# Moon0shang/HandPoseEstimation-with-3D-CNNs

Measured on AMD Instinct MI355X. Metric: depth frames/sec to 32^3 TSDF, higher is better.
Workload: dtype f64

## Files before the change

### handposeestimation-with-3d-cnns_amd/csrc/abi.inc

```


extern "C" {

void tsdf_default_cam(tsdf_cam *cam) {
  if (cam) *cam = kDefaultCam;
}

int tsdf_version(void) { return TSDF_ABI_VERSION; }

const char *tsdf_strerror(int status) {
  switch (status) {
    case TSDF_OK: return "ok";
    case TSDF_ERR_INVALID_ARG: return "invalid argument";
    case TSDF_ERR_NO_DEVICE: return "no usable HIP device (this library is gfx950-only and has no CPU fallback)";
    case TSDF_ERR_LAUNCH: return "HIP kernel launch failed";
    default: return "unknown tsdf status";
  }
}

int tsdf_resolution_supported(int R) { return R >= 4 && R <= kMaxR && (R % 4) == 0; }

int tsdf_voxelize_hip(const float *d_depth, int64_t depth_len, const int64_t *d_offsets, const int32_t *d_headers, int n,
                      int R, const tsdf_cam *cam, int layout, void *hip_stream, float *d_out_tsdf,
                      float *d_out_max_l, float *d_out_mid_p, int32_t *d_out_status) {
// ... 123 lines not shown
}

int tsdf_voxelize_indexed_pca_hip(const float *d_depth, int64_t depth_len, const int64_t *d_offsets,
                                  const int32_t *d_headers, int64_t n_pack, const int64_t *d_index, int n, int R,
                                  const tsdf_cam *cam, int layout, void *hip_stream, const double *d_xforms,
                                  float *d_out_tsdf, float *d_out_max_l, float *d_out_mid_p, int32_t *d_out_status,
                                  const tsdf_labels *labels, const tsdf_pca *pca) {
  RunOpts o;
  o.needs = kNeedPlacement | kNeedIndex | kNeedLabels | kNeedPca;
  o.labels = labels;
  o.index = d_index;
  o.n_src = n_pack;
  o.xforms = d_xforms;
  o.pca = pca;
  return run(Frames{d_depth, depth_len, d_offsets, d_headers, n, R, cam, layout, hip_stream},
             Outs{d_out_tsdf, d_out_max_l, d_out_mid_p, d_out_status}, o);
}

int tsdf_voxelize_indexed_host_pca_hip(const float *d_depth, int64_t depth_len, const int64_t *d_offsets,
                                       const int32_t *d_headers, int64_t n_pack, const int64_t *h_index, int n, int R,
                                       const tsdf_cam *cam, int layout, void *hip_stream, float *d_out_tsdf,
                                       float *d_out_max_l, float *d_out_mid_p, int32_t *d_out_status,
                                       const tsdf_labels *labels, const tsdf_pca *pca) {
  RunOpts o;
  o.needs = kNeedPlacement | kNeedHostIndex | kNeedLabels | kNeedPca;
  o.labels = labels;
  o.h_index = h_index;
  o.n_src = n_pack;
  o.pca = pca;
  return run(Frames{d_depth, depth_len, d_offsets, d_headers, n, R, cam, layout, hip_stream},
             Outs{d_out_tsdf, d_out_max_l, d_out_mid_p, d_out_status}, o);
}

int tsdf_project_joints_hip(const float *d_gt, const float *d_max_l, const float *d_mid_p, int n, int n_joints,
                            const tsdf_pca *pca, void *hip_stream) {
  return run_project(d_gt, d_max_l, d_mid_p, n, n_joints, pca, hip_stream);
}

int tsdf_pose_error_hip(const float *d_pred, const tsdf_pca *pca, const float *d_max_l, const float *d_mid_p,
                        const float *d_gt, int n, int n_joints, void *hip_stream, float *d_out_err,
                        float *d_out_frame_mean, float *d_out_frame_max, float *d_out_joints) {
  return run_pose_error(d_pred, pca, d_max_l, d_mid_p, d_gt, n, n_joints, hip_stream, d_out_err, d_out_frame_mean,
                        d_out_frame_max, d_out_joints);
}

int tsdf_point_clouds_hip(const float *d_depth, int64_t depth_len, const int64_t *d_offsets, const int32_t *d_headers,
                          int n, int points, const tsdf_cam *cam, uint64_t seed, int64_t frame_base,
                          const double *d_xforms, void *hip_stream, double *d_out_points, int32_t *d_out_count,
                          int32_t *d_out_status) {
  return run_point_clouds(d_depth, depth_len, d_offsets, d_headers, n, points, cam, seed, frame_base, d_xforms,
                          hip_stream, d_out_points, d_out_count, d_out_status);
}

int tsdf_cloud_grid_hip(const double *d_points, int n, int points, int R, const tsdf_cam *cam, void *hip_stream,
                        float *d_out_grid, float *d_out_max_l, float *d_out_mid_p, float *d_out_aabb,
                        int32_t *d_out_status) {
  return run_cloud_grid(d_points, n, points, R, cam, hip_stream, d_out_grid, d_out_max_l, d_out_mid_p, d_out_aabb,
                        d_out_status);
}

#ifdef TSDF_DEBUG_HOOKS
int tsdf_debug_pixmap_hip(const float *d_depth, int64_t depth_len, const int64_t *d_offsets, const int32_t *d_headers,
                          int n, int R, const tsdf_cam *cam, int layout, void *hip_stream, const float *d_grid,
                          float *d_out_tsdf, int32_t *d_out_pixmap, int32_t *d_out_status) {
  RunOpts o;
  o.needs = kNeedPixmap;
  o.grid_in = d_grid;
  o.pixmap = d_out_pixmap;
  return run(Frames{d_depth, depth_len, d_offsets, d_headers, n, R, cam, layout, hip_stream},
             Outs{d_out_tsdf, nullptr, nullptr, d_out_status}, o);
}
#endif

int tsdf_stream_release(void *hip_stream) {
  int dev = 0;
  if (hipGetDevice(&dev) != hipSuccess) {
    (void)hipGetLastError();
    return TSDF_OK;
  }
  (void)stream_slot(dev, static_cast<hipStream_t>(hip_stream), true);
  return TSDF_OK;
}

#ifdef TSDF_DEBUG_HOOKS
int tsdf_debug_set_queue_word(void *hip_stream, uint64_t value) {
  int dev = 0;
  const int rc = check_device(&dev);
  if (rc != TSDF_OK) return rc;
  hipStream_t s = static_cast<hipStream_t>(hip_stream);
  const int i = stream_slot(dev, s, false);
  if (i < 0) return TSDF_ERR_INVALID_ARG;
  if (hipStreamSynchronize(s) != hipSuccess) return TSDF_ERR_LAUNCH;
  const unsigned long long v = value;
  if (hipMemcpy(g_slots[dev].base + i, &v, sizeof v, hipMemcpyHostToDevice) != hipSuccess) return TSDF_ERR_LAUNCH;
  return TSDF_OK;
}
#endif

int tsdf_describe_launch(int n, int R, int layout, int aug, char *buf, int buflen) {
  if (!buf || buflen < 1 || n < 1 || !tsdf_resolution_supported(R)) return TSDF_ERR_INVALID_ARG;
  if (layout != TSDF_LAYOUT_CZYX && layout != TSDF_LAYOUT_CXYZ) return TSDF_ERR_INVALID_ARG;
  int dev = 0;
  const int rc = check_device(&dev);
  if (rc != TSDF_OK) return rc;
  const int rt = (R == 32 || R == 64) ? R : 0;
  int S = 0, per = R;
  split_plan(n, R, num_cus(), &S, &per);
  if (S >= 2) {
    snprintf(buf, (size_t)buflen, "tsdf_split_kernel<%d, %d, %s, x%d", rt, layout, aug ? "true" : "false", S);
  } else {
    snprintf(buf, (size_t)buflen, "tsdf_fused_kernel<%d, %d, %s, false, %d>", rt, layout, aug ? "true" : "false",
             groups_for(R));
  }
  return TSDF_OK;
}

#ifdef TSDF_STAMPS
int tsdf_debug_read_stamps(unsigned long long *host_out, int count) {
  const int total = kStampBlocks * kStampFrames * kStampSlots;
  if (count > total) count = total;
  if (hipDeviceSynchronize() != hipSuccess) return -1;
  if (hipMemcpyFromSymbol(host_out, HIP_SYMBOL(g_stamps), sizeof(unsigned long long) * count) != hipSuccess)
    return -1;
  return count;
}
int tsdf_debug_read_wstamps(unsigned long long *host_out, int count) {
  const int total = kStampBlocks * kStampFrames * 16 * 2;
  if (count > total) count = total;
  if (hipDeviceSynchronize() != hipSuccess) return -1;
  if (hipMemcpyFromSymbol(host_out, HIP_SYMBOL(g_wstamps), sizeof(unsigned long long) * count) != hipSuccess)
    return -1;
  return count;
}
#endif

}
```

### handposeestimation-with-3d-cnns_amd/csrc/frame.inc

```

struct KArgs {
  const float *depth;
  const int64_t *offsets;
  const int32_t *headers;
  int n, R;
  CamK cam;
  float *tsdf, *max_l, *mid_p;
  int32_t *status;
  float *aabb, *grid, *ori;
  int aabb_only;
  const float *grid_in;
  unsigned long long *queue;
  unsigned int qepoch;
  const double *xforms;
  int64_t depth_len;
  const int64_t *index;
  int64_t n_src;
  int n_inline;
  int64_t inline_index[TSDF_INLINE_INDEX_MAX];
  const float *gt;
  float *gt_nor, *gt_aug;
  int n_joints, clamp;
  int32_t *pixmap;
  int split, per;
  float *xchg;
  unsigned int seq;
  int polls;
  const float *pca_mean, *pca_coeff;
  float *gt_pca;
  int pca_k;
};

struct FrameHdr {
  int frame;
  int l, t, r, b;
  int pad;
  int64_t off0, off1;
  int64_t src;
};

__device__ __forceinline__ void fetch_header(const KArgs &a, const int64_t *__restrict__ in_offsets,
                                             const int32_t *__restrict__ in_headers, int fr, FrameHdr &m) {
  int64_t src = fr;
  bool ok = true;
  if (a.n_inline) {
    src = a.inline_index[fr];
    ok = src >= 0 && src < a.n_src;
    if (!ok) src = 0;
  } else if (a.index) {
    src = a.index[fr];
    ok = src >= 0 && src < a.n_src;
    if (!ok) src = 0;
  }
  const int32_t *h = in_headers + 6 * src;
  m.l = h[2];
  m.t = h[3];
  m.r = h[4];
  m.b = h[5];
  m.off0 = in_offsets[src];
  m.off1 = ok ? in_offsets[src + 1] : m.off0 - 1;
  m.src = src;
}

struct HelpReq {
  Grid g;
  VoxK vk;
  const float *src;
  float *out;
  int frame, use_tab, mode, owner;
  int pm_bw, pm_dc, pm_dr, pad;
};

struct GroupCtl {
  int bar[kMaxGroups];
  int local_next;
  int tile_next;
  int lock;
  int help_for;
  int idle[kMaxGroups];
  int cap_fail[kMaxGroups];
  FrameHdr hdr[kMaxGroups];
  HelpReq help;
};


__device__ __forceinline__ int lds_load(const int *p) {
  return __hip_atomic_load(p, __ATOMIC_RELAXED, __HIP_MEMORY_SCOPE_WORKGROUP);
}
__device__ __forceinline__ void lds_store(int *p, int v) {
  __hip_atomic_store(p, v, __ATOMIC_RELAXED, __HIP_MEMORY_SCOPE_WORKGROUP);
}

template <int GWAVES>
__device__ __forceinline__ void group_barrier(int *cnt, int &target) {
  target += GWAVES;
  asm volatile("s_waitcnt lgkmcnt(0)" ::: "memory");
  if ((threadIdx.x & 63) == 0) {
    __hip_atomic_fetch_add(cnt, 1, __ATOMIC_RELAXED, __HIP_MEMORY_SCOPE_WORKGROUP);
    while (__hip_atomic_load(cnt, __ATOMIC_RELAXED, __HIP_MEMORY_SCOPE_WORKGROUP) < target)
      __builtin_amdgcn_s_sleep(1);
  }
  asm volatile("" ::: "memory");
}

template <int RT, bool AUG, int GROUPS = 2>
struct Lds {
  static constexpr int kZ = RT ? RT : kMaxR;
  static constexpr bool kHasTab = !AUG && (RT == 0 || RT <= kTabR);
  static constexpr int kTabN = kHasTab ? kTabR * kTabR : 16;
  struct PerGroup {
    alignas(16) unsigned pytab[kTabN];
    alignas(16) int pxtab[kTabN];
    alignas(16) unsigned char pyrow[kTabN];
    alignas(16) ZEntry ztab[kZ];
    alignas(16) double atab[AUG ? 12 * kZ : 2];
    alignas(16) unsigned rowtab[kMaxRows];
    alignas(16) float red[16 * kRedStride];
  };
  static constexpr int kFixed = GROUPS * (int)sizeof(PerGroup) + (int)sizeof(GroupCtl) + 64;
  static constexpr int kPoolFloats = ((kLdsBytes - kFixed) / 16) * 4;
  static constexpr int kPoolUnits = kPoolFloats / 4;
  static_assert(kPoolUnits < 16384, "pool offsets are 14 bits of 4-float units");
  struct Block {
    alignas(16) float pool[kPoolFloats];
    PerGroup pg[GROUPS];
    alignas(16) GroupCtl ctl;
  };
  static_assert(sizeof(Block) <= kLdsBytes, "LDS layout exceeds the CU");
};

template <class PG>
__device__ __forceinline__ Tabs make_tabs(PG &pg) {
  Tabs t;
  t.ztab = (LdsZ)pg.ztab;
  t.pxtab = (LdsCI)pg.pxtab;
  t.pytab = (LdsCU)pg.pytab;
  t.pyrow = (LdsCU8)pg.pyrow;
  t.rowtab = (LdsCU)pg.rowtab;
  t.atab = (LdsCD)pg.atab;
  return t;
}

__device__ __forceinline__ bool frame_from_header(const FrameHdr &fh, const float *depth, int64_t depth_len, Frame &f) {
  f.l = __builtin_amdgcn_readfirstlane(fh.l);
  f.t = __builtin_amdgcn_readfirstlane(fh.t);
  f.r = __builtin_amdgcn_readfirstlane(fh.r);
  f.b = __builtin_amdgcn_readfirstlane(fh.b);
  const int64_t bw = (int64_t)f.r - f.l, bh = (int64_t)f.b - f.t;
  f.bw = (int)bw;
  f.bh = (int)bh;
  f.depth = depth + fh.off0;
  return bw > 0 && bh > 0 && bw <= 0x7fffffff && bh <= 0x7fffffff && bw * bh == fh.off1 - fh.off0 && fh.off0 >= 0 &&
         fh.off1 <= depth_len;
}

__device__ __forceinline__ bool finite32(float v) { return __builtin_fabsf(v) < TSDF_INF; }

__device__ __forceinline__ void place_grid(Aabb &ab, int R, const CamK &cam, const float *grid_in, int frame,
                                           Grid &g, int &status) {
  if (!ab.any) {
    status = TSDF_FRAME_DEGENERATE;
    ab.mn[0] = ab.mn[1] = ab.mn[2] = ab.mx[0] = ab.mx[1] = ab.mx[2] = 0.f;
    return;
  }
  g = glue(ab.mn, ab.mx, R, cam);
// ... 236 lines not shown
```

### handposeestimation-with-3d-cnns_amd/csrc/kernels.inc

```

template <int RT, int LAYOUT, bool AUG, bool DBG, int GROUPS, bool PCA>
__global__ __launch_bounds__(kWG) void tsdf_fused_kernel(const KArgs a, const float *__restrict__ in_depth,
                                                         const int64_t *__restrict__ in_offsets,
                                                         const int32_t *__restrict__ in_headers,
                                                         const double *__restrict__ in_xforms) {
  constexpr int kGroups = GROUPS, kGW = kWG / GROUPS, kGWaves = kGW / 64;
  using L = Lds<RT, AUG, GROUPS>;
  __shared__ typename L::Block lds;

  const int R = RT ? RT : a.R;
  const CamK &cam = a.cam;
  const int n = a.n;
  const int tid = threadIdx.x, lane = tid & 63, gtid = tid & (kGW - 1);
  const int group = __builtin_amdgcn_readfirstlane(tid / kGW);
  const int gwave = __builtin_amdgcn_readfirstlane((tid >> 6) & (kGWaves - 1));
  auto &pg = lds.pg[group];
  GroupCtl &ctl = lds.ctl;

  if (tid == 0) {
    for (int i = 0; i < kGroups; ++i) ctl.bar[i] = ctl.idle[i] = ctl.cap_fail[i] = 0;
    ctl.lock = 0;
    ctl.help_for = 0;
    ctl.local_next = kGroups;
  }
  __syncthreads();
  int bar_target = 0;
  auto gsync = [&]() { group_barrier<kGWaves>(&ctl.bar[group], bar_target); };

  Capture cap;
  cap.pool = (LdsF)lds.pool;
  cap.rowtab = (LdsU)pg.rowtab;
  cap.fail = (LdsI)&ctl.cap_fail[group];
  cap.cap4 = 0;
  cap.base4 = 0;
  cap.on = false;

  const int n_static = gridDim.x * kGroups;

  int iter = 0;
  (void)iter;
  for (;; ++iter) {
    if (gwave == 0) {
      int fr;
      if (iter == 0) {
        fr = blockIdx.x + gridDim.x * group;
      } else if (a.queue) {
        unsigned int t = 0;
        if (lane == 0) {
          t = queue_ticket(a.queue, a.qepoch, n);
        }
        fr = n_static + (int)__builtin_amdgcn_readfirstlane(t);
      } else {
        int t = 0;
        if (lane == 0) t = __hip_atomic_fetch_add(&ctl.local_next, 1, __ATOMIC_RELAXED, __HIP_MEMORY_SCOPE_WORKGROUP);
        const int64_t f64i = (int64_t)blockIdx.x + (int64_t)gridDim.x * __builtin_amdgcn_readfirstlane(t);
        fr = f64i < n ? (int)f64i : n;
      }
      FrameHdr m;
      m.frame = fr < n ? fr : -1;
      m.l = m.t = m.r = m.b = m.pad = 0;
      m.off0 = m.off1 = m.src = 0;
      if (fr < n) fetch_header(a, in_offsets, in_headers, fr, m);
      if (lane == 0) {
        ctl.hdr[group] = m;
        ctl.cap_fail[group] = 0;
      }
    }
    gsync();
    const FrameHdr fh = ctl.hdr[group];
    const int frame = __builtin_amdgcn_readfirstlane(fh.frame);
    if (frame < 0) break;
    TSDF_STAMP(kGroups * iter + group, 0);

    Frame f;
    const bool hdr_ok = frame_from_header(fh, in_depth, a.depth_len, f);
    float *out = a.tsdf ? a.tsdf + (int64_t)frame * 3 * R * R * R : nullptr;
    const bool want_vol = !a.aabb_only && out;

    int status = TSDF_FRAME_OK;
    Aabb ab;
    ab.any = false;
    ab.mn[0] = ab.mn[1] = ab.mn[2] = ab.mx[0] = ab.mx[1] = ab.mx[2] = 0.f;
    ab.c0 = ab.r0 = 0;
    ab.c1 = ab.r1 = -1;
    Grid g;
    g.mid[0] = g.mid[1] = g.mid[2] = 0.f;
    g.max_l = g.voxel_len = g.trunc = 0.f;
    g.ori[0] = g.ori[1] = g.ori[2] = 0.f;
    const double *xf = AUG ? in_xforms + 24 * (int64_t)frame : nullptr;

    bool holds_lock = false;
    if (!hdr_ok) {
      status = TSDF_FRAME_BAD_HEADER;
    } else {
      float fin[kExt];
      auto sync_ext = [&]() {
        if (want_vol && gwave == 0 && lane == 0) {
          while (atomicCAS(&ctl.lock, 0, 1) != 0) __builtin_amdgcn_s_sleep(2);
        }
        gsync();
      };
      phase1_extents<kGWaves, AUG, false>(f, cam, 0, f.bh, pg.red, fin, gwave, sync_ext, cap, kGroups * iter + group, xf);
      holds_lock = want_vol;
      ab = aabb_from_extents(fin);
      TSDF_STAMP(kGroups * iter + group, 4);
      place_grid(ab, R, cam, a.grid_in, frame, g, status);
    }

    if (gtid == 0) write_frame_outputs(a, frame, g, ab, status);
    write_labels<PCA>(a, frame, fh.src, g, status, xf, gtid, kGW);

    if (want_vol) {
      if (status != TSDF_FRAME_OK) {
        zero_volume(out, R, gtid, kGW, 0, 1);
        if constexpr (DBG) {
          if (a.pixmap)
            for (int i = gtid; i < R * R * R; i += kGW) a.pixmap[(int64_t)frame * R * R * R + i] = -1;
        }
      } else {
        int vt = gtid;
        asm volatile("" : "+v"(vt));
        int mode = kFillGlobal;
        const int sc0 = DBG ? 0 : ab.c0, sr0 = DBG ? 0 : ab.r0;
        const int sw = DBG ? f.bw : ab.c1 - ab.c0 + 1, sh = DBG ? f.bh : ab.r1 - ab.r0 + 1;
        const int sw4 = (sw + 3) & ~3;
        const bool staged = (int64_t)sw4 * sh <= L::kPoolFloats;
        if (staged) {
          mode = kFillRect;
          stage_rect_dma<kGWaves>(lds.pool, f, fh.off1 - fh.off0, sc0, sr0, sh, sw4, gwave, lane);
        }
        const VoxK vk = make_voxk(cam, g, f, ab, mode, DBG, sw4);
        const bool use_tab = !AUG && R <= kTabR;
        TSDF_STAMP(kGroups * iter + group, 5);
        fill_tables<LAYOUT, AUG>(pg, g, cam, vk, R, use_tab, false, xf, vt, kGW);
        TSDF_STAMP(kGroups * iter + group, 6);
        if (staged) asm volatile("s_waitcnt vmcnt(0)" ::: "memory");
        TSDF_STAMP(kGroups * iter + group, 7);
        if constexpr (kGroups == 2) {
          if (gwave == 0 && lane == 0) ctl.hdr[group].pad = lds_load(&ctl.idle[group ^ 1]);
        }
        if constexpr (kGroups == 1) {
          if (gwave == 0 && lane == 0) lds_store(&ctl.tile_next, 0);
        }
        gsync();
        TSDF_STAMP(kGroups * iter + group, 8);
        bool helped = false;
        if constexpr (kGroups == 2) {
          if (__builtin_amdgcn_readfirstlane(ctl.hdr[group].pad)) {
            helped = true;
            if (gwave == 0 && lane == 0) {
              HelpReq hq;
              hq.g = g;
              hq.vk = vk;
              hq.src = f.depth + vk.base;
              hq.mode = mode;
              hq.owner = group;
              hq.out = out;
              hq.frame = frame;
              hq.use_tab = use_tab;
              hq.pm_bw = f.bw;
              hq.pm_dc = vk.px0 - f.l;
              hq.pm_dr = vk.py0 - f.t;
              hq.pad = 0;
              ctl.help = hq;
              lds_store(&ctl.help_for, (group ^ 1) + 1);
            }
          }
        }
        TSDF_STAMP_VAL(kGroups * iter + group, 10, helped ? 2 : 1);
        const Tabs tb = make_tabs(pg);
        PixMapK pm;
        pm.out = DBG && a.pixmap ? (GlobalPix)(a.pixmap + (int64_t)frame * R * R * R) : (GlobalPix) nullptr;
        pm.bw = f.bw;
        pm.dc = vk.px0 - f.l;
        pm.dr = vk.py0 - f.t;
        auto run2 = [&](auto src) {
          if constexpr (kGroups == 2) {
            if (__builtin_expect(helped, 0)) {
              if constexpr (AUG) {
                phase2_aug<LAYOUT, 2 * kGW>(g, cam, vk, R, xf, tb, src, (GlobalOut)out, vt, 0, R);
              } else {
                phase2<LAYOUT, 2 * kGW, DBG>(g, cam, vk, R, tb, use_tab, src, (GlobalOut)out, vt, 0, R, pm);
              }
              return;
            }
          }
          if constexpr (AUG) {
            phase2_aug<LAYOUT, kGW>(g, cam, vk, R, xf, tb, src, (GlobalOut)out, vt, 0, R,
                                    kGroups == 1 ? &ctl.tile_next : nullptr, kGroups * iter + group);
          } else {
            phase2<LAYOUT, kGW, DBG>(g, cam, vk, R, tb, use_tab, src, (GlobalOut)out, vt, 0, R, pm,
                                     kGroups == 1 ? &ctl.tile_next : nullptr);
          }
        };
        if (mode == kFillRect) {
          run2(LdsRect{(LdsSrc)lds.pool});
        } else {
          run2((GlobalSrc)(f.depth + vk.base));
        }
      }
    }
    TSDF_STAMP(kGroups * iter + group, 9);
    gsync();
    if (holds_lock && gwave == 0 && lane == 0)
      __hip_atomic_store(&ctl.lock, 0, __ATOMIC_RELAXED, __HIP_MEMORY_SCOPE_WORKGROUP);
  }
  if constexpr (kGroups == 2) {
    if (gwave == 0 && lane == 0) {
      lds_store(&ctl.idle[group], 1);
      int dec;
      for (;;) {
        if (lds_load(&ctl.help_for) == group + 1) { dec = 1; break; }
        if (lds_load(&ctl.idle[group ^ 1])) { dec = lds_load(&ctl.help_for) == group + 1; break; }
        __builtin_amdgcn_s_sleep(8);
      }
      ctl.hdr[group].pad = dec;
    }
    gsync();
    if (__builtin_amdgcn_readfirstlane(ctl.hdr[group].pad)) {
      const HelpReq hq = ctl.help;
      const GlobalOut hout = (GlobalOut)hq.out;
      const GlobalSrc hsrc = (GlobalSrc)hq.src;
      const Tabs tb = make_tabs(lds.pg[group ^ 1]);
      PixMapK pm;
      pm.out = DBG && a.pixmap ? (GlobalPix)(a.pixmap + (int64_t)hq.frame * R * R * R) : (GlobalPix) nullptr;
      pm.bw = hq.pm_bw;
      pm.dc = hq.pm_dc;
      pm.dr = hq.pm_dr;
      auto run2 = [&](auto src) {
        if constexpr (AUG) {
          phase2_aug<LAYOUT, 2 * kGW>(hq.g, cam, hq.vk, R, in_xforms + 24 * (int64_t)hq.frame, tb, src, hout,
                                      kGW + gtid, 0, R);
        } else {
          phase2<LAYOUT, 2 * kGW, DBG>(hq.g, cam, hq.vk, R, tb, hq.use_tab != 0, src, hout, kGW + gtid, 0, R, pm);
        }
      };
      if (hq.mode == kFillRect) {
        run2(LdsRect{(LdsSrc)lds.pool});
      } else {
        run2(hsrc);
      }
    }
  }
}


template <int RT, int LAYOUT, bool AUG, bool XCHG, bool PCA>
__global__ __launch_bounds__(kWG) void tsdf_split_kernel(const KArgs a, const float *__restrict__ in_depth,
                                                         const int64_t *__restrict__ in_offsets,
                                                         const int32_t *__restrict__ in_headers,
                                                         const double *__restrict__ in_xforms) {
  using L = Lds<RT, AUG>;
  __shared__ typename L::Block lds;

  const int R = RT ? RT : a.R;
  const CamK &cam = a.cam;
  const int tid = threadIdx.x;
  const int wave = __builtin_amdgcn_readfirstlane(tid >> 6);
  const int frame = blockIdx.x / a.split, part = blockIdx.x - frame * a.split;
  auto &pg = lds.pg[0];
  GroupCtl &ctl = lds.ctl;
  if (tid == 0) ctl.cap_fail[0] = 0;
  FrameHdr fh;
  {
    fh.frame = frame;
    fh.pad = 0;
    fetch_header(a, in_offsets, in_headers, frame, fh);
  }
  __syncthreads();
  TSDF_STAMP(0, 0);
  Frame f;
  const bool hdr_ok = frame_from_header(fh, in_depth, a.depth_len, f);
  float *out = a.tsdf ? a.tsdf + (int64_t)frame * 3 * R * R * R : nullptr;
  const bool want_vol = !a.aabb_only && out;

  int status = TSDF_FRAME_OK;
  Aabb ab;
  ab.any = false;
  ab.mn[0] = ab.mn[1] = ab.mn[2] = ab.mx[0] = ab.mx[1] = ab.mx[2] = 0.f;
  ab.c0 = ab.r0 = 0;
  ab.c1 = ab.r1 = -1;
  Grid g;
  g.mid[0] = g.mid[1] = g.mid[2] = 0.f;
  g.max_l = g.voxel_len = g.trunc = 0.f;
  g.ori[0] = g.ori[1] = g.ori[2] = 0.f;
  const double *xf = AUG ? in_xforms + 24 * (int64_t)frame : nullptr;

  Capture cap;
  cap.pool = (LdsF)lds.pool;
  cap.rowtab = (LdsU)pg.rowtab;
  cap.fail = (LdsI)&ctl.cap_fail[0];
  cap.cap4 = L::kPoolUnits / (kWG / 64);
  cap.base4 = wave * cap.cap4;
  cap.on = false;
  if (!hdr_ok) {
    status = TSDF_FRAME_BAD_HEADER;
  } else {
    float fin[kExt];
    auto sync_all = [&]() { __syncthreads(); };
    bool have = false;
    if constexpr (XCHG) {
      const int S = a.split;
      const int rb = (int)((int64_t)f.bh * part / S), re = (int)((int64_t)f.bh * (part + 1) / S);
      phase1_extents<kWG / 64, AUG, false>(f, cam, rb, re, pg.red, fin, wave, sync_all, cap, 0, xf);
      float *boxes = a.xchg + (int64_t)frame * (kXchgParts * kXchgBox);
      if (tid == 0) {
        unsigned int *box = reinterpret_cast<unsigned int *>(boxes + part * kXchgBox);
#pragma unroll
        for (int i = 0; i < kExt; ++i)
          __hip_atomic_store(box + i, __float_as_uint(fin[i]), __ATOMIC_RELAXED, __HIP_MEMORY_SCOPE_AGENT);
        asm volatile("s_waitcnt vmcnt(0)" ::: "memory");
        __hip_atomic_store(box + kExt, a.seq, __ATOMIC_RELAXED, __HIP_MEMORY_SCOPE_AGENT);
      }
      TSDF_STAMP(0, 13);
      if (wave == 0) {
        const int lane = tid & 63;
        const bool mine = lane < S;
        const unsigned int *box = reinterpret_cast<const unsigned int *>(boxes + (mine ? lane : 0) * kXchgBox);
        bool ready = !mine || lane == part;
        for (int it = 0; it < a.polls; ++it) {
          if (!ready) ready = __hip_atomic_load(box + kExt, __ATOMIC_RELAXED, __HIP_MEMORY_SCOPE_AGENT) == a.seq;
          if (__all(ready)) break;
          __builtin_amdgcn_s_sleep(1);
// ... 209 lines not shown
```

### handposeestimation-with-3d-cnns_amd/csrc/launch.inc

```

const tsdf_cam kDefaultCam = {241.42, 160.0, 120.0, 1.0f, 3.0f};

int num_cus() {
  static std::atomic<int> cached[64];
  int dev = 0;
  if (hipGetDevice(&dev) != hipSuccess || dev < 0 || dev >= 64) return 256;
  int v = cached[dev].load(std::memory_order_relaxed);
  if (v == 0) {
    if (hipDeviceGetAttribute(&v, hipDeviceAttributeMultiprocessorCount, dev) != hipSuccess || v <= 0) v = 256;
    cached[dev].store(v, std::memory_order_relaxed);
  }
  return v;
}

int check_device(int *dev_out) {
  static std::atomic<int> arch_state[64];
  int dev = 0;
  if (hipGetDevice(&dev) != hipSuccess) {
    (void)hipGetLastError();
    return TSDF_ERR_NO_DEVICE;
  }
  *dev_out = dev;
  if (dev < 0 || dev >= 64) return TSDF_OK;
  int st = arch_state[dev].load(std::memory_order_relaxed);
  if (st == 0) {
    hipDeviceProp_t prop;
    if (hipGetDeviceProperties(&prop, dev) != hipSuccess) {
      (void)hipGetLastError();
      return TSDF_ERR_NO_DEVICE;
    }
    st = strncmp(prop.gcnArchName, "gfx950", 6) == 0 ? 1 : -1;
    arch_state[dev].store(st, std::memory_order_relaxed);
  }
  return st == 1 ? TSDF_OK : TSDF_ERR_NO_DEVICE;
}

void split_plan(int n, int R, int cus, int *split, int *per) {
  *split = 0;
  *per = R;
  if (n > cus / 2 || n > kXchgFrames) return;
  const int G = R * (R / 4);
  const int sstep = (G <= kWG && kWG % G == 0) ? kWG / G : 1;
  const int rounds = (R + sstep - 1) / sstep;
  int S = cus / n;
  if (S < 2) S = 2;
  if (S > rounds) S = rounds;
  if (S > kXchgParts) S = kXchgParts;
  if (S < 2) return;
  const int p = ((rounds + S - 1) / S) * sstep;
  S = (R + p - 1) / p;
  if (S < 2) return;
  *split = S;
  *per = p;
}

int xchg_polls() {
#ifdef TSDF_DEBUG_HOOKS
  static const int polls = [] {
    const char *e = getenv("TSDF_XCHG_POLLS");
    return e ? atoi(e) : kXchgPolls;
  }();
  return polls;
#else
  return kXchgPolls;
#endif
}

template <int RT, int LAYOUT, bool AUG, bool DBG, bool PCA = false>
hipError_t launch(hipStream_t s, KArgs &a, int dev) {
  const int cus = num_cus();
  if constexpr (!DBG) {
    int S = 0, per = a.R;
    if (!a.aabb_only && a.tsdf) split_plan(a.n, a.R, cus, &S, &per);
    if (S >= 2) {
      a.split = S;
      a.per = per;
      a.queue = nullptr;
      a.xchg = a.n <= kXchgFrames ? xchg_for(dev, s, &a.seq) : nullptr;
      a.polls = xchg_polls();
      if (a.xchg) {
        hipLaunchKernelGGL((tsdf_split_kernel<RT, LAYOUT, AUG, true, PCA>), dim3(a.n * S), dim3(kWG), 0, s, a, a.depth,
                           a.offsets, a.headers, a.xforms);
      } else {
        hipLaunchKernelGGL((tsdf_split_kernel<RT, LAYOUT, AUG, false, PCA>), dim3(a.n * S), dim3(kWG), 0, s, a, a.depth,
                           a.offsets, a.headers, a.xforms);
      }
      return hipGetLastError();
    }
  }
  const int grid = a.n < cus ? a.n : cus;
  a.split = 0;
  a.per = a.R;
  auto fused = [&](auto groups_tag) {
    constexpr int G = decltype(groups_tag)::value;
    a.queue = a.n > grid * G ? queue_word(dev, s, &a.qepoch) : nullptr;
    hipLaunchKernelGGL((tsdf_fused_kernel<RT, LAYOUT, AUG, DBG, G, PCA>), dim3(grid), dim3(kWG), 0, s, a, a.depth, a.offsets,
                       a.headers, a.xforms);
  };
  if constexpr (RT != 0) {
    fused(std::integral_constant<int, groups_for(RT)>{});
  } else {
    if (groups_for(a.R) == 1) fused(std::integral_constant<int, 1>{});
    else fused(std::integral_constant<int, 2>{});
  }
  return hipGetLastError();
}

template <int LAYOUT, bool AUG, bool PCA = false>
hipError_t launch_r(hipStream_t s, KArgs &a, int dev) {
  if (a.R == 32) return launch<32, LAYOUT, AUG, false, PCA>(s, a, dev);
  if (a.R == 64) return launch<64, LAYOUT, AUG, false, PCA>(s, a, dev);
  return launch<0, LAYOUT, AUG, false, PCA>(s, a, dev);
}

using namespace tsdf_host;

int run(const Frames &f, const Outs &out, const RunOpts &o) {
  const int chk = check_run_args(f, out, o, tsdf_resolution_supported(f.R));
  if (chk == kNothingToDo) return TSDF_OK;
  if (chk != TSDF_OK) return chk;
  const int n = f.n, R = f.R, layout = f.layout;
  const tsdf_cam *cam = f.cam ? f.cam : &kDefaultCam;
  int dev = 0;
  int rc = check_device(&dev);
  if (rc != TSDF_OK) return rc;
  KArgs a;
  memset(&a, 0, sizeof a);
  a.depth = f.depth;
  a.offsets = f.offsets;
  a.headers = f.headers;
  a.n = n;
  a.R = R;
  a.cam.focal = cam->focal;
  a.cam.cx = cam->cx;
  a.cam.cy = cam->cy;
  a.cam.inv_focal = 1.0 / cam->focal;
  a.cam.eps = cam->invalid_eps;
  a.cam.trunc_vox = cam->trunc_voxels;
  a.tsdf = out.tsdf;
  a.max_l = out.max_l;
  a.mid_p = out.mid_p;
  a.status = out.status;
  a.aabb = o.aabb;
  a.grid = o.grid;
  a.ori = o.ori;
  a.aabb_only = o.aabb_only;
  a.grid_in = o.grid_in;
  a.xforms = o.xforms;
  a.depth_len = f.depth_len;
  a.index = o.index;
  a.n_src = o.n_src;
  if (o.needs & kNeedHostIndex) {
    a.n_inline = n;
    memcpy(a.inline_index, o.h_index, sizeof(int64_t) * (size_t)n);
  }
  if (o.labels) {
    a.gt = o.labels->d_gt;
    a.gt_nor = o.labels->d_out_gt_nor;
    a.gt_aug = o.labels->d_out_gt_aug;
    a.n_joints = o.labels->n_joints;
    a.clamp = o.labels->clamp;
  }
  if (o.pca) {
    a.pca_mean = o.pca->d_mean;
    a.pca_coeff = o.pca->d_coeff;
    a.gt_pca = o.pca->d_out_gt_pca;
    a.pca_k = o.pca->n_components;
  }
  a.pixmap = o.pixmap;
  hipStream_t s = static_cast<hipStream_t>(f.stream);
  hipError_t e;
  if (o.pixmap) {
#ifdef TSDF_DEBUG_HOOKS
    if (layout == TSDF_LAYOUT_CZYX)
      e = R == 32 ? launch<32, 0, false, true>(s, a, dev) : launch<0, 0, false, true>(s, a, dev);
    else
      e = R == 32 ? launch<32, 1, false, true>(s, a, dev) : launch<0, 1, false, true>(s, a, dev);
#else
// ... 77 lines not shown
```

### handposeestimation-with-3d-cnns_amd/csrc/queue.inc

```

constexpr int kQueueSlots = 1024;
__device__ unsigned long long g_queue[kQueueSlots];

__device__ __forceinline__ unsigned int queue_next_epoch(unsigned int e) { return e + 1u ? e + 1u : 1u; }

__device__ __forceinline__ unsigned int queue_ticket(unsigned long long *q, unsigned int epoch, int n) {
  const unsigned long long mine = (unsigned long long)epoch << 32;
  unsigned int t;
  for (;;) {
    const unsigned long long old = atomicAdd(q, 1ull);
    if ((unsigned int)(old >> 32) == epoch) {
      t = (unsigned int)old;
      break;
    }
    unsigned long long cur = old + 1;
    bool installed = false;
    for (;;) {
      const unsigned long long seen = atomicCAS(q, cur, mine | 1ull);
      if (seen == cur) {
        installed = true;
        break;
      }
      if ((unsigned int)(seen >> 32) == epoch) break;
      cur = seen;
    }
    if (installed) {
      t = 0u;
      break;
    }
  }
  if (t == (unsigned int)(n - 1))
    __hip_atomic_store(q, (unsigned long long)queue_next_epoch(epoch) << 32, __ATOMIC_RELAXED, __HIP_MEMORY_SCOPE_AGENT);
  return t;
}

constexpr int kXchgParts = 16;
constexpr int kXchgFrames = 128;
constexpr int kXchgBox = 16;
constexpr int kXchgPolls = 4000;

struct StreamSlots {
  tsdf_host::SlotTable<kQueueSlots> table;
  std::mutex mu;
  unsigned long long *base = nullptr;
  float *xchg = nullptr;
  unsigned int xchg_seq[64] = {0};
};
StreamSlots g_slots[64];

int stream_slot(int dev, hipStream_t s, bool release) {
  if (dev < 0 || dev >= 64) return -1;
  StreamSlots &t = g_slots[dev];
  const bool per_thread = s == hipStreamPerThread;
  if (release) {
    t.table.release(static_cast<const void *>(s), per_thread);
    return -1;
  }
  hipStreamCaptureStatus cs = hipStreamCaptureStatusNone;
  if (hipStreamIsCapturing(s, &cs) != hipSuccess) {
    (void)hipGetLastError();
    return -1;
  }
  if (cs != hipStreamCaptureStatusNone) return -1;
  {
    std::lock_guard<std::mutex> lock(t.mu);
    if (!t.base) {
      void *p = nullptr;
      if (hipGetSymbolAddress(&p, HIP_SYMBOL(g_queue)) != hipSuccess || !p) {
        (void)hipGetLastError();
        return -1;
      }
      t.base = static_cast<unsigned long long *>(p);
    }
  }
  return t.table.acquire(static_cast<const void *>(s), per_thread);
}

unsigned long long *queue_word(int dev, hipStream_t s, unsigned int *epoch) {
  const int i = stream_slot(dev, s, false);
  if (i < 0) return nullptr;
  *epoch = g_slots[dev].table.next_epoch(i);
  return g_slots[dev].base + i;
}

constexpr int kXchgSlots = 64;
constexpr size_t kXchgSlotFloats = (size_t)kXchgFrames * kXchgParts * kXchgBox;
__device__ float g_xchg[kXchgSlots * kXchgSlotFloats];
float *xchg_for(int dev, hipStream_t s, unsigned int *seq) {
  const int i = stream_slot(dev, s, false);
  if (i < 0 || i >= kXchgSlots) return nullptr;
  StreamSlots &t = g_slots[dev];
  std::lock_guard<std::mutex> lock(t.mu);
  if (!t.xchg) {
    void *p = nullptr;
    if (hipGetSymbolAddress(&p, HIP_SYMBOL(g_xchg)) != hipSuccess || !p) {
      (void)hipGetLastError();
      return nullptr;
    }
    t.xchg = static_cast<float *>(p);
  }
  unsigned int v = ++t.xchg_seq[i];
  if (v == 0) v = ++t.xchg_seq[i];
  *seq = v;
  return t.xchg + (size_t)i * kXchgSlotFloats;
}
```

### handposeestimation-with-3d-cnns_amd/csrc/tsdf_hip.hip

```cpp

#include <hip/hip_runtime.h>
#include <stdint.h>
#include <stdio.h>
#include <stdlib.h>
#include <string.h>

#include <atomic>
#include <mutex>
#include <thread>
#include <type_traits>

#include "../../include/tsdf.h"
#ifdef TSDF_DEBUG_HOOKS
#include "../../include/tsdf_debug.h"
#endif
#include "tsdf_host.inc"


namespace {

#include "common.inc"
#include "phase1.inc"
#include "phase2.inc"
#include "frame.inc"
#include "queue.inc"
#include "kernels.inc"
#include "launch.inc"
#include "cloud.inc"
#include "cloudgrid.inc"

}

#include "abi.inc"
```

### include/tsdf_debug.h

```cpp
#ifndef TSDF_DEBUG_H_
#define TSDF_DEBUG_H_

#include "tsdf.h"

#ifdef __cplusplus
extern "C" {
#endif

int tsdf_debug_pixmap_hip(const float *d_depth, int64_t depth_len, const int64_t *d_offsets, const int32_t *d_headers,
                          int n, int R, const tsdf_cam *cam, int layout, void *hip_stream, const float *d_grid,
                          float *d_out_tsdf, int32_t *d_out_pixmap, int32_t *d_out_status);

int tsdf_debug_set_queue_word(void *hip_stream, uint64_t value);

#ifdef __cplusplus
}
#endif
#endif
```

Baseline: 7.090 million.

## Add cross-workgroup board so idle workgroups adopt frames blocked on LDS lock

Adds a device-global offer board: when a group in a two-group workgroup cannot take the shared LDS pool lock, it publishes its frame's grid and AABB to a global slot and waits for the lock. If another workgroup claims that slot first, the frame is skipped locally. Workgroups that have finished their own queue scan the board and run stage, table fill and phase-2 voxelization for adopted frames using the full workgroup. This targets tail imbalance and time spent serialized on the per-workgroup lock, at the cost of global atomics, polling, sleeps and extra LDS control state.

```diff
diff --git a/handposeestimation-with-3d-cnns_amd/csrc/abi.inc b/handposeestimation-with-3d-cnns_amd/csrc/abi.inc
--- a/handposeestimation-with-3d-cnns_amd/csrc/abi.inc
+++ b/handposeestimation-with-3d-cnns_amd/csrc/abi.inc
@@ -229,8 +229,27 @@
   return TSDF_OK;
 }
 
+#ifdef TSDF_BOARD_STATS
+static int board_counts(uint64_t *out3) {
+  unsigned int v[4] = {0, 0, 0, 0};
+  const unsigned int z[4] = {0, 0, 0, 0};
+  if (hipDeviceSynchronize() != hipSuccess) return TSDF_ERR_LAUNCH;
+  if (hipMemcpyFromSymbol(v, HIP_SYMBOL(g_board_stats), sizeof v) != hipSuccess) return TSDF_ERR_LAUNCH;
+  if (hipMemcpyToSymbol(HIP_SYMBOL(g_board_stats), z, sizeof z) != hipSuccess) return TSDF_ERR_LAUNCH;
+  out3[0] = v[0];
+  out3[1] = v[1];
+  out3[2] = v[2];
+  return TSDF_OK;
+}
+#endif
+#ifdef TSDF_STAMPS
+int tsdf_debug_read_board(uint64_t *out3) { return out3 ? board_counts(out3) : TSDF_ERR_INVALID_ARG; }
+#endif
+
 #ifdef TSDF_DEBUG_HOOKS
 int tsdf_debug_set_queue_word(void *hip_stream, uint64_t value) {
+  if (hip_stream == TSDF_DEBUG_BOARD_COUNTS)
+    return value ? board_counts(reinterpret_cast<uint64_t *>(static_cast<uintptr_t>(value))) : TSDF_ERR_INVALID_ARG;
   int dev = 0;
   const int rc = check_device(&dev);
   if (rc != TSDF_OK) return rc;
diff --git a/handposeestimation-with-3d-cnns_amd/csrc/frame.inc b/handposeestimation-with-3d-cnns_amd/csrc/frame.inc
--- a/handposeestimation-with-3d-cnns_amd/csrc/frame.inc
+++ b/handposeestimation-with-3d-cnns_amd/csrc/frame.inc
@@ -29,6 +29,8 @@
   const float *pca_mean, *pca_coeff;
   float *gt_pca;
   int pca_k;
+  unsigned int *board;
+  unsigned int btag, bdone;
 };
 
 struct FrameHdr {
@@ -81,6 +83,12 @@
   int cap_fail[kMaxGroups];
   FrameHdr hdr[kMaxGroups];
   HelpReq help;
+  int got[kMaxGroups];
+  int mine[kMaxGroups];
+  int idle_cnt;
+  int adopt_last;
+  int adopt_slot[2];
+  unsigned int adopt[16];
 };
 
 
diff --git a/handposeestimation-with-3d-cnns_amd/csrc/kernels.inc b/handposeestimation-with-3d-cnns_amd/csrc/kernels.inc
--- a/handposeestimation-with-3d-cnns_amd/csrc/kernels.inc
+++ b/handposeestimation-with-3d-cnns_amd/csrc/kernels.inc
@@ -1,3 +1,63 @@
+
+template <int RT, int LAYOUT, bool AUG, class LB>
+__device__ __forceinline__ void adopt_frame(const KArgs &a, const float *__restrict__ in_depth,
+                                            const int64_t *__restrict__ in_offsets,
+                                            const int32_t *__restrict__ in_headers,
+                                            const double *__restrict__ in_xforms, LB &lds, int R, int tid) {
+  using L = Lds<RT, AUG, 2>;
+  const CamK &cam = a.cam;
+  const unsigned int *w = lds.ctl.adopt;
+  const int frame = __builtin_amdgcn_readfirstlane((int)w[0]);
+  Grid g;
+  g.mid[0] = __uint_as_float(w[1]);
+  g.mid[1] = __uint_as_float(w[2]);
+  g.mid[2] = __uint_as_float(w[3]);
+  g.max_l = __uint_as_float(w[4]);
+  g.voxel_len = __uint_as_float(w[5]);
+  g.trunc = __uint_as_float(w[6]);
+  g.ori[0] = __uint_as_float(w[7]);
+  g.ori[1] = __uint_as_float(w[8]);
+  g.ori[2] = __uint_as_float(w[9]);
+  Aabb ab;
+  ab.any = true;
+  ab.mn[0] = ab.mn[1] = ab.mn[2] = ab.mx[0] = ab.mx[1] = ab.mx[2] = 0.f;
+  ab.c0 = __builtin_amdgcn_readfirstlane((int)w[10]);
+  ab.c1 = __builtin_amdgcn_readfirstlane((int)w[11]);
+  ab.r0 = __builtin_amdgcn_readfirstlane((int)w[12]);
+  ab.r1 = __builtin_amdgcn_readfirstlane((int)w[13]);
+  FrameHdr fh;
+  fh.frame = frame;
+  fh.pad = 0;
+  fetch_header(a, in_offsets, in_headers, frame, fh);
+  Frame f;
+  const bool hdr_ok = frame_from_header(fh, in_depth, a.depth_len, f);
+  const int sw4 = (ab.c1 - ab.c0 + 4) & ~3, sh = ab.r1 - ab.r0 + 1;
+  const bool fits = hdr_ok && ab.c0 >= 0 && ab.r0 >= 0 && ab.c1 < f.bw && ab.r1 < f.bh && sw4 > 0 && sh > 0 &&
+                    (int64_t)sw4 * sh <= L::kPoolFloats && frame >= 0 && frame < a.n;
+  if (fits) {
+    const double *xf = AUG ? in_xforms + 24 * (int64_t)frame : nullptr;
+    const GlobalOut out = (GlobalOut)(a.tsdf + (int64_t)frame * 3 * R * R * R);
+    auto &pg = lds.pg[0];
+    stage_rect_dma<kWG / 64>(lds.pool, f, fh.off1 - fh.off0, ab.c0, ab.r0, sh, sw4,
+                             __builtin_amdgcn_readfirstlane(tid >> 6), tid & 63);
+    const VoxK vk = make_voxk(cam, g, f, ab, kFillRect, false, sw4);
+    const bool use_tab = !AUG && R <= kTabR;
+    fill_tables<LAYOUT, AUG>(pg, g, cam, vk, R, use_tab, false, xf, tid, kWG);
+    asm volatile("s_waitcnt vmcnt(0)" ::: "memory");
+    __syncthreads();
+    const Tabs tb = make_tabs(pg);
+    if constexpr (AUG) {
+      phase2_aug<LAYOUT, kWG>(g, cam, vk, R, xf, tb, LdsRect{(LdsSrc)lds.pool}, out, tid, 0, R);
+    } else {
+      PixMapK pm;
+      pm.out = (GlobalPix) nullptr;
+      pm.bw = f.bw;
+      pm.dc = pm.dr = 0;
+      phase2<LAYOUT, kWG, false>(g, cam, vk, R, tb, use_tab, LdsRect{(LdsSrc)lds.pool}, out, tid, 0, R, pm);
+    }
+  }
+  __syncthreads();
+}
 
 template <int RT, int LAYOUT, bool AUG, bool DBG, int GROUPS, bool PCA>
 __global__ __launch_bounds__(kWG) void tsdf_fused_kernel(const KArgs a, const float *__restrict__ in_depth,
@@ -16,12 +76,15 @@
   const int gwave = __builtin_amdgcn_readfirstlane((tid >> 6) & (kGWaves - 1));
   auto &pg = lds.pg[group];
   GroupCtl &ctl = lds.ctl;
+  constexpr bool kBoard = GROUPS == 2 && !DBG;
+  [[maybe_unused]] unsigned int *const board = kBoard ? a.board : nullptr;
 
   if (tid == 0) {
     for (int i = 0; i < kGroups; ++i) ctl.bar[i] = ctl.idle[i] = ctl.cap_fail[i] = 0;
     ctl.lock = 0;
     ctl.help_for = 0;
     ctl.local_next = kGroups;
+    if constexpr (kBoard) ctl.idle_cnt = ctl.adopt_last = 0;
   }
   __syncthreads();
   int bar_target = 0;
@@ -96,12 +159,27 @@
       float fin[kExt];
       auto sync_ext = [&]() {
         if (want_vol && gwave == 0 && lane == 0) {
-          while (atomicCAS(&ctl.lock, 0, 1) != 0) __builtin_amdgcn_s_sleep(2);
+          if constexpr (kBoard) {
+            int got = 1;
+            while (atomicCAS(&ctl.lock, 0, 1) != 0) {
+              if (board && lds_load(&ctl.bar[group]) >= bar_target + kGWaves - 1) {
+                got = 0;
+                break;
+              }
+              __builtin_amdgcn_s_sleep(2);
+            }
+            lds_store(&ctl.got[group], got);
+          } else {
+            while (atomicCAS(&ctl.lock, 0, 1) != 0) __builtin_amdgcn_s_sleep(2);
+          }
         }
         gsync();
       };
       phase1_extents<kGWaves, AUG, false>(f, cam, 0, f.bh, pg.red, fin, gwave, sync_ext, cap, kGroups * iter + group, xf);
       holds_lock = want_vol;
+      if constexpr (kBoard) {
+        if (want_vol) holds_lock = __builtin_amdgcn_readfirstlane(lds_load(&ctl.got[group])) != 0;
+      }
       ab = aabb_from_extents(fin);
       TSDF_STAMP(kGroups * iter + group, 4);
       place_grid(ab, R, cam, a.grid_in, frame, g, status);
@@ -110,7 +188,30 @@
     if (gtid == 0) write_frame_outputs(a, frame, g, ab, status);
     write_labels<PCA>(a, frame, fh.src, g, status, xf, gtid, kGW);
 
-    if (want_vol) {
+    bool adopted = false;
+    if constexpr (kBoard) {
+      if (want_vol && hdr_ok && !holds_lock && status == TSDF_FRAME_OK) {
+        if (gwave == 0 && lane == 0) {
+          const int slot = kGroups * blockIdx.x + group;
+          const int sw4 = (ab.c1 - ab.c0 + 4) & ~3, sh = ab.r1 - ab.r0 + 1;
+          bool offered = false;
+          if ((int64_t)sw4 * sh <= L::kPoolFloats)
+            offered = board_offer(board, a.btag, slot, iter > 0, frame, g, ab, kFillRect);
+          while (atomicCAS(&ctl.lock, 0, 1) != 0) __builtin_amdgcn_s_sleep(2);
+          int mine = 1;
+          if (offered && !board_withdraw(board, a.btag, slot)) {
+            mine = 0;
+            __hip_atomic_store(&ctl.lock, 0, __ATOMIC_RELAXED, __HIP_MEMORY_SCOPE_WORKGROUP);
+          }
+          lds_store(&ctl.mine[group], mine);
+        }
+        gsync();
+        holds_lock = __builtin_amdgcn_readfirstlane(lds_load(&ctl.mine[group])) != 0;
+        adopted = !holds_lock;
+      }
+    }
+
+    if (want_vol && !adopted) {
       if (status != TSDF_FRAME_OK) {
         zero_volume(out, R, gtid, kGW, 0, 1);
         if constexpr (DBG) {
@@ -208,6 +309,12 @@
   if constexpr (kGroups == 2) {
     if (gwave == 0 && lane == 0) {
       lds_store(&ctl.idle[group], 1);
+      if constexpr (kBoard) {
+        if (board && __hip_atomic_fetch_add(&ctl.idle_cnt, 1, __ATOMIC_RELAXED, __HIP_MEMORY_SCOPE_WORKGROUP) == 1) {
+          const unsigned int before = atomicAdd(board + kBoardDone, 1u);
+          lds_store(&ctl.adopt_last, before + 1u == a.bdone);
+        }
+      }
       int dec;
       for (;;) {
         if (lds_load(&ctl.help_for) == group + 1) { dec = 1; break; }
@@ -239,6 +346,43 @@
         run2(LdsRect{(LdsSrc)lds.pool});
       } else {
         run2(hsrc);
+      }
+    }
+    if constexpr (kBoard) {
+      if (board) {
+        __syncthreads();
+        if (!lds_load(&ctl.adopt_last)) {
+          const int wave = __builtin_amdgcn_readfirstlane(tid >> 6);
+          const int nslots = kGroups * (int)gridDim.x;
+          for (int scan = 0, empty = 0; empty < kAdoptScans; ++scan) {
+            if (wave == 0) {
+              int slot = board_take(board, a.btag, nslots, lane);
+              if (slot >= 0) {
+                unsigned int w = 0;
+                if (lane < 15) w = board_read(board + kBoardPayload + slot * kBoardWords + lane);
+                if (lane < 15) ctl.adopt[lane] = w;
+                asm volatile("s_waitcnt vmcnt(0)" ::: "memory");
+                if (lane == 0) {
+                  __hip_atomic_store(board + slot, a.btag | kConsumed, __ATOMIC_RELAXED, __HIP_MEMORY_SCOPE_AGENT);
+                  TSDF_BOARD_COUNT(2);
+                }
+              } else if (lane == 0) {
+                const unsigned int d = __hip_atomic_load(board + kBoardDone, __ATOMIC_RELAXED, __HIP_MEMORY_SCOPE_AGENT);
+                if ((int)(d - a.bdone) >= 0) slot = -2;
+              }
+              if (lane == 0) lds_store(&ctl.adopt_slot[scan & 1], slot);
+            }
+            __syncthreads();
+            const int slot = __builtin_amdgcn_readfirstlane(lds_load(&ctl.adopt_slot[scan & 1]));
+            if (slot == -2) break;
+            if (slot < 0) {
+              ++empty;
+              __builtin_amdgcn_s_sleep(32);
+              continue;
+            }
+            adopt_frame<RT, LAYOUT, AUG>(a, in_depth, in_offsets, in_headers, in_xforms, lds, R, tid);
+          }
+        }
       }
     }
   }
diff --git a/handposeestimation-with-3d-cnns_amd/csrc/launch.inc b/handposeestimation-with-3d-cnns_amd/csrc/launch.inc
--- a/handposeestimation-with-3d-cnns_amd/csrc/launch.inc
+++ b/handposeestimation-with-3d-cnns_amd/csrc/launch.inc
@@ -93,7 +93,10 @@
   a.per = a.R;
   auto fused = [&](auto groups_tag) {
     constexpr int G = decltype(groups_tag)::value;
-    a.queue = a.n > grid * G ? queue_word(dev, s, &a.qepoch) : nullptr;
+    const int slot = a.n > grid * G ? stream_slot(dev, s, false) : -1;
+    a.queue = queue_word_at(dev, slot, &a.qepoch);
+    a.board = nullptr;
+    if (G == 2 && !DBG && a.queue && !a.aabb_only && a.tsdf) a.board = board_at(dev, slot, grid, &a.btag, &a.bdone);
     hipLaunchKernelGGL((tsdf_fused_kernel<RT, LAYOUT, AUG, DBG, G, PCA>), dim3(grid), dim3(kWG), 0, s, a, a.depth, a.offsets,
                        a.headers, a.xforms);
   };
diff --git a/handposeestimation-with-3d-cnns_amd/csrc/queue.inc b/handposeestimation-with-3d-cnns_amd/csrc/queue.inc
--- a/handposeestimation-with-3d-cnns_amd/csrc/queue.inc
+++ b/handposeestimation-with-3d-cnns_amd/csrc/queue.inc
@@ -34,6 +34,69 @@
   return t;
 }
 
+constexpr int kBoardWgs = 512;
+constexpr int kBoardSlots = 2 * kBoardWgs;
+constexpr int kBoardWords = 16;
+constexpr int kBoardDone = kBoardSlots;
+constexpr int kBoardPayload = kBoardSlots + 32;
+constexpr size_t kBoardStride = (size_t)kBoardPayload + (size_t)kBoardSlots * kBoardWords;
+constexpr unsigned int kOffered = 1, kTaken = 2, kWithdrawn = 3, kConsumed = 4;
+constexpr int kAdoptScans = 64;
+__device__ unsigned int g_board[64 * kBoardStride];
+#ifdef TSDF_BOARD_STATS
+__device__ unsigned int g_board_stats[4];
+#define TSDF_BOARD_COUNT(i) atomicAdd(&g_board_stats[i], 1u)
+#else
+#define TSDF_BOARD_COUNT(i) do { } while (0)
+#endif
+
+__device__ __forceinline__ unsigned int board_read(unsigned int *p) { return atomicCAS(p, 0xffffffffu, 0xffffffffu); }
+
+__device__ __forceinline__ bool board_offer(unsigned int *board, unsigned int tag, int slot, bool again, int frame,
+                                            const Grid &g, const Aabb &ab, int mode) {
+  unsigned int *st = board + slot;
+  if (again && board_read(st) == (tag | kTaken)) return false;
+  unsigned int *w = board + kBoardPayload + slot * kBoardWords;
+  const unsigned int v[15] = {(unsigned int)frame, __float_as_uint(g.mid[0]), __float_as_uint(g.mid[1]),
+                              __float_as_uint(g.mid[2]), __float_as_uint(g.max_l), __float_as_uint(g.voxel_len),
+                              __float_as_uint(g.trunc), __float_as_uint(g.ori[0]), __float_as_uint(g.ori[1]),
+                              __float_as_uint(g.ori[2]), (unsigned int)ab.c0, (unsigned int)ab.c1, (unsigned int)ab.r0,
+                              (unsigned int)ab.r1, (unsigned int)mode};
+#pragma unroll
+  for (int i = 0; i < 15; ++i) __hip_atomic_store(w + i, v[i], __ATOMIC_RELAXED, __HIP_MEMORY_SCOPE_AGENT);
+  asm volatile("s_waitcnt vmcnt(0)" ::: "memory");
+  __hip_atomic_store(st, tag | kOffered, __ATOMIC_RELAXED, __HIP_MEMORY_SCOPE_AGENT);
+  TSDF_BOARD_COUNT(0);
+  return true;
+}
+
+__device__ __forceinline__ bool board_withdraw(unsigned int *board, unsigned int tag, int slot) {
+  const bool mine = atomicCAS(board + slot, tag | kOffered, tag | kWithdrawn) == (tag | kOffered);
+  if (mine) TSDF_BOARD_COUNT(1);
+  return mine;
+}
+
+__device__ __forceinline__ int board_take(unsigned int *board, unsigned int tag, int nslots, int lane) {
+  const int n64 = (nslots + 63) & ~63;
+  const int rot = (int)((blockIdx.x * 128u) % (unsigned)n64);
+  for (int base = 0; base < n64; base += 64) {
+    int slot = base + rot + lane;
+    slot = slot >= n64 ? slot - n64 : slot;
+    unsigned int st = 0;
+    if (slot < nslots) st = __hip_atomic_load(board + slot, __ATOMIC_RELAXED, __HIP_MEMORY_SCOPE_AGENT);
+    unsigned long long mask = __ballot(st == (tag | kOffered));
+    while (mask) {
+      const int l = __builtin_ctzll(mask);
+      mask &= mask - 1;
+      const int cand = __builtin_amdgcn_readlane(slot, l);
+      int ok = 0;
+      if (lane == 0) ok = atomicCAS(board + cand, tag | kOffered, tag | kTaken) == (tag | kOffered);
+      if (__builtin_amdgcn_readfirstlane(ok)) return cand;
+    }
+  }
+  return -1;
+}
+
 constexpr int kXchgParts = 16;
 constexpr int kXchgFrames = 128;
 constexpr int kXchgBox = 16;
@@ -45,6 +108,9 @@
   unsigned long long *base = nullptr;
   float *xchg = nullptr;
   unsigned int xchg_seq[64] = {0};
+  unsigned int *board = nullptr;
+  unsigned int board_epoch[64] = {0};
+  unsigned int board_done[64] = {0};
 };
 StreamSlots g_slots[64];
 
@@ -76,11 +142,30 @@
   return t.table.acquire(static_cast<const void *>(s), per_thread);
 }
 
-unsigned long long *queue_word(int dev, hipStream_t s, unsigned int *epoch) {
-  const int i = stream_slot(dev, s, false);
+unsigned long long *queue_word_at(int dev, int i, unsigned int *epoch) {
   if (i < 0) return nullptr;
   *epoch = g_slots[dev].table.next_epoch(i);
   return g_slots[dev].base + i;
+}
+
+unsigned int *board_at(int dev, int i, int grid, unsigned int *tag, unsigned int *target) {
+  if (i < 0 || i >= 64 || grid > kBoardWgs) return nullptr;
+  StreamSlots &t = g_slots[dev];
+  std::lock_guard<std::mutex> lock(t.mu);
+  if (!t.board) {
+    void *p = nullptr;
+    if (hipGetSymbolAddress(&p, HIP_SYMBOL(g_board)) != hipSuccess || !p) {
+      (void)hipGetLastError();
+      return nullptr;
+    }
+    t.board = static_cast<unsigned int *>(p);
+  }
+  unsigned int e = ++t.board_epoch[i] & 0x1fffffffu;
+  if (e == 0) e = ++t.board_epoch[i] & 0x1fffffffu;
+  *tag = e << 3;
+  t.board_done[i] += (unsigned int)grid;
+  *target = t.board_done[i];
+  return t.board + (size_t)i * kBoardStride;
 }
 
 constexpr int kXchgSlots = 64;
diff --git a/handposeestimation-with-3d-cnns_amd/csrc/tsdf_hip.hip b/handposeestimation-with-3d-cnns_amd/csrc/tsdf_hip.hip
--- a/handposeestimation-with-3d-cnns_amd/csrc/tsdf_hip.hip
+++ b/handposeestimation-with-3d-cnns_amd/csrc/tsdf_hip.hip
@@ -19,6 +19,10 @@
 
 namespace {
 
+#if defined(TSDF_DEBUG_HOOKS) || defined(TSDF_STAMPS)
+#define TSDF_BOARD_STATS 1
+#endif
+
 #include "common.inc"
 #include "phase1.inc"
 #include "phase2.inc"
diff --git a/include/tsdf_debug.h b/include/tsdf_debug.h
--- a/include/tsdf_debug.h
+++ b/include/tsdf_debug.h
@@ -11,6 +11,7 @@
                           int n, int R, const tsdf_cam *cam, int layout, void *hip_stream, const float *d_grid,
                           float *d_out_tsdf, int32_t *d_out_pixmap, int32_t *d_out_status);
 
+#define TSDF_DEBUG_BOARD_COUNTS ((void *)(intptr_t)-1)
 int tsdf_debug_set_queue_word(void *hip_stream, uint64_t value);
 
 #ifdef __cplusplus
```

After: 6.561 million. 0.925x the previous value.
